# jdeschut/tunempc

Hardware: AMD Instinct MI355X
Metric: stage-Hessian convexifications/sec at (nx+nu)=32, p=64 (higher is better)
Workload: dtype f64

## Files before the change

### tunempc_amd/csrc/tmpc_cr.h

```cpp
#pragma once
#include <climits>
#include <vector>

#include "tmpc_common.h"
#include "tmpc_factor.h"
#include "tmpc_gemm_dma.h"

namespace tmpc {

constexpr int CR_EW = 8;
constexpr int CR_UW = 8;
enum { CE_NODE = 0, CE_NA, CE_NB, CE_EA, CE_EB, CE_FILL, CE_FX, CE_FACC };
enum { CU_NODE = 0, CU_E0, CU_S0, CU_E1, CU_S1 };

struct CrLevel { int eoff, nelim, uoff, nupd; };
struct CrSched {
  int p = 0;
  int prep = 0;
  std::vector<int> orient;
  std::vector<int> elim, upd;
  std::vector<CrLevel> lev;
};

static inline CrSched cr_build(int p) {
// ... 161 lines not shown
  const int* er = cr.elim + (size_t)(eoff + g % nelim) * CR_EW;
  const int which = r / nstrip, strip = r - which * nstrip;
  const int slot = which ? er[CE_EB] : er[CE_EA];
  if (slot < 0) return;
  const int node = er[CE_NODE], dp = dm.dp;
  const size_t bs = (size_t)dp * dp;
  const double* Dk = w.D + ((size_t)b * dm.p + node) * bs;
  const double* Li = w.Linv + ((size_t)b * dm.p + node) * dm.nt * TB * TB;
  const int r0 = strip * rs;
  const int rows = (dp - r0 < rs) ? dp - r0 : rs;
  double* X = cr_edge(w, dm, b, slot) + (size_t)r0 * dp;
  int jt = 0;
  for (int j0 = 0; j0 < dp; j0 += TB, ++jt) {
    const int nb = (dp - j0 < TB) ? dp - j0 : TB;
    if (j0 > 0) wg_gemm_nt<USE_MFMA, 2, 2, 2, NS>(X + j0, dp, X, dp, Dk + (size_t)j0 * dp, dp, rows, nb, j0, GM_SUB, false, lds);
    wg_gemm_nt<USE_MFMA, 2, 2, 2, NS>(X + j0, dp, X + j0, dp, Li + (size_t)jt * TB * TB, TB, rows, nb, nb, GM_SET, false, lds);
  }
}

constexpr int TRR_NT = 5;
__device__ __forceinline__ void vm_wait_le(int n) {
#define TMPC_VMW(K) case K / 2: asm volatile("s_waitcnt vmcnt(" #K ") lgkmcnt(0)" ::: "memory"); break;
  switch (n >> 1) {
    TMPC_VMW(0) TMPC_VMW(2) TMPC_VMW(4) TMPC_VMW(6) TMPC_VMW(8) TMPC_VMW(10) TMPC_VMW(12) TMPC_VMW(14) TMPC_VMW(16) TMPC_VMW(18) TMPC_VMW(20) TMPC_VMW(22)
    default: asm volatile("s_waitcnt vmcnt(24) lgkmcnt(0)" ::: "memory"); break;
  }
#undef TMPC_VMW
}
#ifndef TMPC_TRD_DEPTH
#define TMPC_TRD_DEPTH 2
#endif
constexpr int TRD_DEPTH = TMPC_TRD_DEPTH;
constexpr int trd_lds_doubles() { return 4 * 1024 + TRD_DEPTH * 2048; }
template <bool POTRF>
__device__ __forceinline__ void trd_strip(double* X, const double* Dk, const double* Li, int rows, int nt, int dp, int it, double* lds, float* X32 = nullptr, int ld32 = 0) {
  constexpr int FR = 4, RS = 16 * FR, ASL = RS * 16, DP = TRD_DEPTH;
  int tid = threadIdx.x;
  if (POTRF) asm volatile("" : "+v"(tid));
  const int lane = tid & 63, wv = __builtin_amdgcn_readfirstlane(tid >> 6);
  const int ws = (wv + it) & 3, wc0 = ws * 16;
  const int fk = lane >> 4, fq = (lane >> 2) & 3, fj = lane & 3;
  const int i1 = (rows + 15) >> 4;
  const int nlast = nt - 1, nbl = (dp - 64 * nlast < 64) ? dp - 64 * nlast : 64, ncl = nbl >> 4;
  const int ntd = POTRF ? nt - 1 : nt;
  const bool rw = ws < i1;
  double* At = lds;
  double* Bs = lds + 4 * ASL;
  unsigned voT[2], voL[2];
#pragma unroll
  for (int h = 0; h < 2; ++h) {
    const int row = wv * 16 + 8 * h + (lane >> 3), c = lane & 7;
    voT[h] = (unsigned)(row * TB + 2 * (c ^ dma_sw(row))) * 8u;
    voL[h] = (unsigned)(row * dp + 2 * (c ^ dma_sw(row))) * 8u;
  }
  int oa[2], ob[4][2];
  {
    const int swa = dma_sw(4 * fq + fj);
#pragma unroll
    for (int hh = 0; hh < 2; ++hh) oa[hh] = (4 * fq + fj) * 16 + 2 * ((4 * hh + fk) ^ swa);
#pragma unroll
    for (int e = 0; e < 4; ++e) {
      const int swb = dma_sw(4 * fj + e);
#pragma unroll
      for (int hh = 0; hh < 2; ++hh) ob[e][hh] = (4 * fj + e) * 16 + 2 * ((4 * hh + fk) ^ swb);
    }
  }
  double acc0[4][4], acc1[4][4], acc2[4][4], acc3[4][4];
  int vmtot = 0, vmk0 = 0, vmk1 = 0, vmk2 = 0;
#define TRD_NB(T) ((dp - 64 * (T) < 64) ? dp - 64 * (T) : 64)
// ... 11 lines not shown
    if (on_) vmtot += 2 * i1;                                                                               \
  }
#define TRD_LOAD_R(I, NC, SET)                                                                              \
  {                                                                                                         \
    _Pragma("unroll") for (int c = 0; c < 4; ++c) {                                                          \
      double2_t u0 = (double2_t){0.0, 0.0}, u1 = u0;                                                        \
      if (rw && c < (NC)) {                                                                                 \
        gcptr2 cp = (gcptr2)(X + (size_t)(wc0 + 4 * fq + fk) * dp + 64 * (I) + 16 * c + 4 * fj);            \
        u0 = cp[0]; u1 = cp[1];                                                                             \
      }                                                                                                     \
      SET[c][0] = -u0[0]; SET[c][1] = -u0[1]; SET[c][2] = -u1[0]; SET[c][3] = -u1[1];                       \
    }                                                                                                       \
    if (rw) vmtot += 2 * (NC);                                                                              \
  }
#define TRD_STORE_R(I, NC, SET, SG)                                                                         \
  if (rw) {                                                                                                 \
    _Pragma("unroll") for (int c = 0; c < 4; ++c) {                                                          \
      if (c < (NC)) {                                                                                       \
        typedef double2_t __attribute__((address_space(1)))* gptr2;                                         \
        gptr2 cp = (gptr2)(X + (size_t)(wc0 + 4 * fq + fk) * dp + 64 * (I) + 16 * c + 4 * fj);              \
        if (X32) {       \
          typedef float4_t __attribute__((address_space(1)))* gptr4;                                        \
          *(gptr4)(X32 + (size_t)(wc0 + 4 * fq + fk) * ld32 + 64 * (I) + 16 * c + 4 * fj) =                 \
              (float4_t){(float)(SG SET[c][0]), (float)(SG SET[c][1]), (float)(SG SET[c][2]), (float)(SG SET[c][3])}; \
        } else {                                                                                            \
          cp[0] = (double2_t){SG SET[c][0], SG SET[c][1]}; cp[1] = (double2_t){SG SET[c][2], SG SET[c][3]}; \
        }                                                                                                   \
      }                                                                                                     \
    }                                                                                                       \
    vmtot += (X32 ? 1 : 2) * (NC);                                                                          \
  }
#define TRD_PARK_C(SET)                                                                        \
  {                                                                                                         \
    _Pragma("unroll") for (int i = 0; i < 4; ++i) {                                                          \
      const int row = 16 * i + 4 * fq + fk, sw_ = dma_sw(row);                                              \
      double* q = At + ws * ASL + row * 16;                                                                \
      *(double2_t*)(q + 2 * ((2 * fj) ^ sw_)) = (double2_t){-SET[i][0], -SET[i][1]};                        \
      *(double2_t*)(q + 2 * ((2 * fj + 1) ^ sw_)) = (double2_t){-SET[i][2], -SET[i][3]};                    \
    }                                                                                                       \
  }
#define TRD_PARK_R(NC, SET, SG)                                                                             \
  if (rw) {                                                                                                 \
    const int row = wc0 + 4 * fq + fk, sw_ = dma_sw(row);                                                   \
    _Pragma("unroll") for (int c = 0; c < 4; ++c) {                                                          \
      if (c < (NC)) {                                                                                       \
        double* q = At + c * ASL + row * 16;                                                               \
        *(double2_t*)(q + 2 * ((2 * fj) ^ sw_)) = (double2_t){SG SET[c][0], SG SET[c][1]};                  \
        *(double2_t*)(q + 2 * ((2 * fj + 1) ^ sw_)) = (double2_t){SG SET[c][2], SG SET[c][3]};              \
      }                                                                                                     \
    }                                                                                                       \
  }
#define TRD_ZERO(SET)                                                                                       \
  {                                                                                                         \
    _Pragma("unroll") for (int i = 0; i < 4; ++i)                                                            \
      _Pragma("unroll") for (int c = 0; c < 4; ++c) SET[i][c] = 0.0;                                        \
  }
  int ii = 0, ij = 0, is = 0, nissued = 0, ndone = 0;
#define TRD_ISSUE()           \
  {                                                                                                         \
    if (ii < ntd) {                                                                                         \
      double* dst_ = Bs + (nissued % DP) * 2048 + wv * 256;                                                 \
      const int nsl_ = (ij == ii) ? (TRD_NB(ii) >> 4) : 4;                                                  \
      const bool two_ = 2 * is + 1 < nsl_;                                                                  \
      if (ij == ii) {                                                                                       \
        const int nb_ = TRD_NB(ii);                                                                         \
        const __amdgpu_buffer_rsrc_t rs_ = __builtin_amdgcn_make_buffer_rsrc((void*)(Li + (size_t)ii * TB * TB), 0, (int)(((unsigned)(nb_ - 1) * TB + (unsigned)nb_) * 8u), 0x00020000); \
        __builtin_amdgcn_raw_ptr_buffer_load_lds(rs_, (lds_vptr)(dst_), 16, voT[0], is * 256, 0, 0);        \
        __builtin_amdgcn_raw_ptr_buffer_load_lds(rs_, (lds_vptr)(dst_ + 128), 16, voT[1], is * 256, 0, 0);  \
        if (two_) {                                                                                         \
          __builtin_amdgcn_raw_ptr_buffer_load_lds(rs_, (lds_vptr)(dst_ + 1024), 16, voT[0], is * 256 + 128, 0, 0);       \
          __builtin_amdgcn_raw_ptr_buffer_load_lds(rs_, (lds_vptr)(dst_ + 1024 + 128), 16, voT[1], is * 256 + 128, 0, 0); \
        }                                                                                                   \
      } else {                                                                                              \
        const int nb_ = TRD_NB(ij);                                                                         \
        const __amdgpu_buffer_rsrc_t rs_ = __builtin_amdgcn_make_buffer_rsrc((void*)(Dk + (size_t)(64 * ij) * dp + 64 * ii), 0, (int)(((unsigned)(nb_ - 1) * (unsigned)dp + 64u) * 8u), 0x00020000); \
        __builtin_amdgcn_raw_ptr_buffer_load_lds(rs_, (lds_vptr)(dst_), 16, voL[0], is * 256, 0, 0);        \
        __builtin_amdgcn_raw_ptr_buffer_load_lds(rs_, (lds_vptr)(dst_ + 128), 16, voL[1], is * 256, 0, 0);  \
        __builtin_amdgcn_raw_ptr_buffer_load_lds(rs_, (lds_vptr)(dst_ + 1024), 16, voL[0], is * 256 + 128, 0, 0);         \
        __builtin_amdgcn_raw_ptr_buffer_load_lds(rs_, (lds_vptr)(dst_ + 1024 + 128), 16, voL[1], is * 256 + 128, 0, 0);   \
      }                                                                                                     \
      vmtot += (ij == ii && !two_) ? 2 : 4;                                                                 \
      { const int k_ = nissued % DP; if (k_ == 0) vmk0 = vmtot; else if (k_ == 1) vmk1 = vmtot; else vmk2 = vmtot; }  \
      ++nissued;                                                                                            \
      if (++is == ((nsl_ + 1) >> 1)) { is = 0; if (++ij >= ntd) { ++ii; ij = ii; } }                        \
    }                                                                                                       \
  }
#define TRD_MMA_C(TGT, AS, BS)                                                                              \
  _Pragma("unroll") for (int hh = 0; hh < 2; ++hh) {                                                        \
    double2_t a_[4], b_[4];                                                                                  \
    _Pragma("unroll") for (int i = 0; i < 4; ++i) a_[i] = *(const double2_t*)((AS) + oa[hh] + i * 256);      \
    _Pragma("unroll") for (int cb = 0; cb < 4; ++cb) b_[cb] = *(const double2_t*)((BS) + wc0 * 16 + ob[cb][hh]); \
    _Pragma("unroll") for (int i = 0; i < 4; ++i) {                                                          \
      _Pragma("unroll") for (int cb = 0; cb < 4; ++cb) {                                                    \
        TGT[i][cb] = __builtin_amdgcn_mfma_f64_4x4x4f64(a_[i][0], b_[cb][0], TGT[i][cb], 0, 0, 0);          \
        TGT[i][cb] = __builtin_amdgcn_mfma_f64_4x4x4f64(a_[i][1], b_[cb][1], TGT[i][cb], 0, 0, 0);          \
      }                                                                                                     \
    }                                                                                                       \
  }
#define TRD_MMA_R(TGT, AS, BS, C0, NC)                                                                      \
  _Pragma("unroll") for (int hh = 0; hh < 2; ++hh) {                                                        \
    const double2_t a_ = *(const double2_t*)((AS) + oa[hh] + wc0 * 16);                                     \
    _Pragma("unroll") for (int c = 0; c < 4; ++c) {                                                          \
      if (c >= (C0) && c < (NC)) {                                                                          \
        double2_t b_[4];                                                                                     \
        _Pragma("unroll") for (int cb = 0; cb < 4; ++cb) b_[cb] = *(const double2_t*)((BS) + c * 256 + ob[cb][hh]); \
        _Pragma("unroll") for (int cb = 0; cb < 4; ++cb) {                                                  \
          TGT[c][cb] = __builtin_amdgcn_mfma_f64_4x4x4f64(a_[0], b_[cb][0], TGT[c][cb], 0, 0, 0);           \
          TGT[c][cb] = __builtin_amdgcn_mfma_f64_4x4x4f64(a_[1], b_[cb][1], TGT[c][cb], 0, 0, 0);           \
        }                                                                                                   \
      }                                                                                                     \
    }                                                                                                       \
  }
#define TRD_STEP_C(TGT) { TRD_MMA_C(TGT, A0, Bc) TRD_MMA_C(TGT, A0 + ASL, Bc + 1024) }
#define TRD_STEP_D0(TGT) { TRD_MMA_R(TGT, At, Bc, 0, 4) TRD_MMA_R(TGT, At + ASL, Bc + 1024, 1, 4) }
#define TRD_STEP_D1(TGT) { TRD_MMA_R(TGT, At + 2 * ASL, Bc, 2, 4) TRD_MMA_R(TGT, At + 3 * ASL, Bc + 1024, 3, 4) }
#define TRD_STEP_RL(N) { TRD_MMA_R(acc0, A0, Bc, 0, N) TRD_MMA_R(acc0, A0 + ASL, Bc + 1024, 0, N) }

  __syncthreads();
  TMPC_TC0()
  TRD_ISSUE()
  if (DP > 2) TRD_ISSUE()
  TRD_LOAD_C(0, acc0)
  if (nt > 2) TRD_LOAD_C(1, acc1) else TRD_ZERO(acc1)
  if (nt > 3) TRD_LOAD_C(2, acc2) else TRD_ZERO(acc2)
  if (nt > 4) TRD_LOAD_C(3, acc3) else TRD_ZERO(acc3)
// ... 93 lines not shown
#undef TRD_STEP_C
#undef TRD_MMA_R
#undef TRD_MMA_C
#undef TRD_ISSUE
#undef TRD_ZERO
#undef TRD_PARK_R
#undef TRD_PARK_C
#undef TRD_STORE_R
#undef TRD_LOAD_R
#undef TRD_LOAD_C
#undef TRD_NB
}

__global__ void __launch_bounds__(256, 2) k_cr_trsm_dma(WS w, Dims dm, CrDev cr, int eoff, int nelim, int count) {
  const int dp = dm.dp;
  const int nst = (dp + 63) / 64;
  const int per = 2 * nst;
  const int it = cr_item(count * nelim * per);
  if (it < 0) return;
  extern __shared__ __attribute__((aligned(16))) double lds[];
  const int g = it / per, r = it - g * per;
  const int b = cr.alist[g / nelim];
  const int* er = cr.elim + (size_t)(eoff + g % nelim) * CR_EW;
  const int which = r / nst, strip = r - which * nst;
  const int slot = which ? er[CE_EB] : er[CE_EA];
  if (slot < 0) return;
  const int node = er[CE_NODE];
  const double* Dk = w.D + ((size_t)b * dm.p + node) * (size_t)dp * dp;
  const double* Li = w.Linv + ((size_t)b * dm.p + node) * dm.nt * TB * TB;
  const int r0 = strip * 64;
  const bool lp = cr_lowp(w, b);
  if (lp && (dm.flags & DF_LOWP_TRSM)) return;
  const int ld32 = cr_ld32(dm);
  trd_strip<false>(cr_edge(w, dm, b, slot) + (size_t)r0 * dp, Dk, Li, (dp - r0 < 64) ? dp - r0 : 64, dm.nt, dp, it, lds,
                   lp ? cr_edge32(w, dm, b, slot) + (size_t)r0 * ld32 : nullptr, ld32);
}

constexpr int trf_lds_doubles() { return 2048 + TRD_DEPTH * 2048; }
__device__ __forceinline__ void trf_strip(const double* X, const double* Dk, const double* Li, int rows, int nt, int dp, int it, double* lds, float* X32, int ld32) {
  constexpr int ASL = 64 * 16, DP = TRD_DEPTH;
  const int tid = threadIdx.x;
  const int lane = tid & 63, wv = __builtin_amdgcn_readfirstlane(tid >> 6);
  const int ws = (wv + it) & 3, wc0 = ws * 16;
  const int fk = lane >> 4, fr = lane & 15;
  const int i1 = (rows + 15) >> 4;
  const int nlast = nt - 1, nbl = (dp - 64 * nlast < 64) ? dp - 64 * nlast : 64, ncl = nbl >> 4;
  const int ntd = nt;
  const bool rw = ws < i1;
  float* At = (float*)lds;
  double* Bs = lds + 2048;
  unsigned voT[2], voL[2];
#pragma unroll
  for (int h = 0; h < 2; ++h) {
    const int row = wv * 16 + 8 * h + (lane >> 3), c = lane & 7;
    voT[h] = (unsigned)(row * TB + 2 * (c ^ dma_sw(row))) * 8u;
    voL[h] = (unsigned)(row * dp + 2 * (c ^ dma_sw(row))) * 8u;
  }
  int of[2];
#pragma unroll
  for (int hh = 0; hh < 2; ++hh) of[hh] = fr * 16 + 2 * ((4 * hh + fk) ^ dma_sw(fr));
  const int asw = (fr >> 1) & 3, ofa = fr * 16 + 4 * (fk ^ asw);
  const int opa0 = 4 * ((2 * fk) & 3 ^ asw) + 2 * (fk >> 1), opa1 = 4 * ((2 * fk + 1) & 3 ^ asw) + 2 * (fk >> 1);
  float4_t acc0[4], acc1[4], acc2[4], acc3[4];
  int vmtot = 0, vmk0 = 0, vmk1 = 0, vmk2 = 0;
#define TRF_NB(T) ((dp - 64 * (T) < 64) ? dp - 64 * (T) : 64)
#define TRF_LOAD_C(I, SET)                                                                                  \
  {                                                                                                         \
    const bool on_ = wc0 < TRF_NB(I);                                                                       \
    _Pragma("unroll") for (int i = 0; i < 4; ++i) {                                                          \
      double2_t u0 = (double2_t){0.0, 0.0}, u1 = u0;                                                        \
      if (on_ && i < i1) {                                                                                  \
        gcptr2 cp = (gcptr2)(X + (size_t)(16 * i + fr) * dp + 64 * (I) + wc0 + 4 * fk);                     \
        u0 = cp[0]; u1 = cp[1];                                                                             \
      }                                                                                                     \
      SET[i] = (float4_t){(float)-u0[0], (float)-u0[1], (float)-u1[0], (float)-u1[1]};                      \
    }                                                                                                       \
    if (on_) vmtot += 2 * i1;                                                                               \
  }
#define TRF_LOAD_R(I, NC, SET)                                                                              \
  {                                                                                                         \
    _Pragma("unroll") for (int c = 0; c < 4; ++c) {                                                          \
      double2_t u0 = (double2_t){0.0, 0.0}, u1 = u0;                                                        \
      if (rw && c < (NC)) {                                                                                 \
        gcptr2 cp = (gcptr2)(X + (size_t)(wc0 + fr) * dp + 64 * (I) + 16 * c + 4 * fk);                     \
        u0 = cp[0]; u1 = cp[1];                                                                             \
      }                                                                                                     \
      SET[c] = (float4_t){(float)-u0[0], (float)-u0[1], (float)-u1[0], (float)-u1[1]};                      \
    }                                                                                                       \
    if (rw) vmtot += 2 * (NC);                                                                              \
  }
#define TRF_STORE_R(I, NC, SET)                                                                             \
  if (rw) {                                                                                                 \
    typedef float4_t __attribute__((address_space(1)))* gptr4;                                              \
    _Pragma("unroll") for (int c = 0; c < 4; ++c)                                                            \
      if (c < (NC)) *(gptr4)(X32 + (size_t)(wc0 + fr) * ld32 + 64 * (I) + 16 * c + 4 * fk) = SET[c];        \
    vmtot += (NC);                                                                                          \
  }
#define TRF_PARK_C(SET)                                                                        \
  {                                                                                                         \
    _Pragma("unroll") for (int i = 0; i < 4; ++i) {                                                          \
      float* q = At + ws * ASL + (16 * i + fr) * 16;                                                        \
      *(float2_t*)(q + opa0) = (float2_t){-SET[i][0], -SET[i][1]};                                           \
      *(float2_t*)(q + opa1) = (float2_t){-SET[i][2], -SET[i][3]};                                           \
    }                                                                                                       \
  }
#define TRF_PARK_R(NC, SET, SG)                                                                             \
  if (rw) {                                                                                                 \
    _Pragma("unroll") for (int c = 0; c < 4; ++c) {                                                          \
      if (c < (NC)) {                                                                                       \
        float* q = At + c * ASL + (wc0 + fr) * 16;                                                          \
        *(float2_t*)(q + opa0) = (float2_t){SG SET[c][0], SG SET[c][1]};                                     \
        *(float2_t*)(q + opa1) = (float2_t){SG SET[c][2], SG SET[c][3]};                                     \
      }                                                                                                     \
    }                                                                                                       \
  }
#define TRF_ZERO(SET) { _Pragma("unroll") for (int i = 0; i < 4; ++i) SET[i] = (float4_t){0.f, 0.f, 0.f, 0.f}; }
  int ii = 0, ij = 0, is = 0, nissued = 0, ndone = 0;
#define TRF_ISSUE()                                                       \
  {                                                                                                         \
    if (ii < ntd) {                                                                                         \
      double* dst_ = Bs + (nissued % DP) * 2048 + wv * 256;                                                 \
      const int nsl_ = (ij == ii) ? (TRF_NB(ii) >> 4) : 4;                                                  \
      const bool two_ = 2 * is + 1 < nsl_;                                                                  \
      if (ij == ii) {                                                                                       \
        const int nb_ = TRF_NB(ii);                                                                         \
        const __amdgpu_buffer_rsrc_t rs_ = __builtin_amdgcn_make_buffer_rsrc((void*)(Li + (size_t)ii * TB * TB), 0, (int)(((unsigned)(nb_ - 1) * TB + (unsigned)nb_) * 8u), 0x00020000); \
        __builtin_amdgcn_raw_ptr_buffer_load_lds(rs_, (lds_vptr)(dst_), 16, voT[0], is * 256, 0, 0);        \
        __builtin_amdgcn_raw_ptr_buffer_load_lds(rs_, (lds_vptr)(dst_ + 128), 16, voT[1], is * 256, 0, 0);  \
        if (two_) {                                                                                         \
          __builtin_amdgcn_raw_ptr_buffer_load_lds(rs_, (lds_vptr)(dst_ + 1024), 16, voT[0], is * 256 + 128, 0, 0);       \
          __builtin_amdgcn_raw_ptr_buffer_load_lds(rs_, (lds_vptr)(dst_ + 1024 + 128), 16, voT[1], is * 256 + 128, 0, 0); \
        }                                                                                                   \
      } else {                                                                                              \
        const int nb_ = TRF_NB(ij);                                                                         \
        const __amdgpu_buffer_rsrc_t rs_ = __builtin_amdgcn_make_buffer_rsrc((void*)(Dk + (size_t)(64 * ij) * dp + 64 * ii), 0, (int)(((unsigned)(nb_ - 1) * (unsigned)dp + 64u) * 8u), 0x00020000); \
        __builtin_amdgcn_raw_ptr_buffer_load_lds(rs_, (lds_vptr)(dst_), 16, voL[0], is * 256, 0, 0);        \
        __builtin_amdgcn_raw_ptr_buffer_load_lds(rs_, (lds_vptr)(dst_ + 128), 16, voL[1], is * 256, 0, 0);  \
        __builtin_amdgcn_raw_ptr_buffer_load_lds(rs_, (lds_vptr)(dst_ + 1024), 16, voL[0], is * 256 + 128, 0, 0);         \
        __builtin_amdgcn_raw_ptr_buffer_load_lds(rs_, (lds_vptr)(dst_ + 1024 + 128), 16, voL[1], is * 256 + 128, 0, 0);   \
      }                                                                                                     \
      vmtot += (ij == ii && !two_) ? 2 : 4;                                                                 \
      { const int k_ = nissued % DP; if (k_ == 0) vmk0 = vmtot; else if (k_ == 1) vmk1 = vmtot; else vmk2 = vmtot; }  \
      ++nissued;                                                                                            \
      if (++is == ((nsl_ + 1) >> 1)) { is = 0; if (++ij >= ntd) { ++ii; ij = ii; } }                        \
    }                                                                                                       \
  }
#define TRF_MMA_C(TGT, AS, BS)                                                                              \
  {                                                                                                         \
    float4_t a_[4];                                                                                          \
    _Pragma("unroll") for (int i = 0; i < 4; ++i) a_[i] = *(const float4_t*)((AS) + i * 256 + ofa);         \
    _Pragma("unroll") for (int hh = 0; hh < 2; ++hh) {                                                      \
      const double2_t b_ = *(const double2_t*)((BS) + wc0 * 16 + of[hh]);                                   \
      _Pragma("unroll") for (int e = 0; e < 2; ++e) {                                                        \
        const float bf_ = (float)b_[e];                                                                      \
        _Pragma("unroll") for (int i = 0; i < 4; ++i)                                                        \
          TGT[i] = __builtin_amdgcn_mfma_f32_16x16x4f32(bf_, a_[i][2 * hh + e], TGT[i], 0, 0, 0);           \
      }                                                                                                     \
    }                                                                                                       \
  }
#define TRF_MMA_R(TGT, AS, BS, C0, NC)                                                                      \
  {                                                                                                         \
    const float4_t a_ = *(const float4_t*)((AS) + wc0 * 16 + ofa);                                          \
    _Pragma("unroll") for (int hh = 0; hh < 2; ++hh) {                                                      \
      double2_t b_[4];                                                                                       \
      _Pragma("unroll") for (int c = 0; c < 4; ++c)                                                          \
        if (c >= (C0) && c < (NC)) b_[c] = *(const double2_t*)((BS) + c * 256 + of[hh]);                    \
      _Pragma("unroll") for (int e = 0; e < 2; ++e) {                                                        \
        _Pragma("unroll") for (int c = 0; c < 4; ++c)                                                        \
          if (c >= (C0) && c < (NC)) TGT[c] = __builtin_amdgcn_mfma_f32_16x16x4f32((float)b_[c][e], a_[2 * hh + e], TGT[c], 0, 0, 0); \
      }                                                                                                     \
    }                                                                                                       \
  }
#define TRF_STEP_C(TGT) { TRF_MMA_C(TGT, A0, Bc) TRF_MMA_C(TGT, A0 + ASL, Bc + 1024) }
#define TRF_STEP_D0(TGT) { TRF_MMA_R(TGT, At, Bc, 0, 4) TRF_MMA_R(TGT, At + ASL, Bc + 1024, 1, 4) }
#define TRF_STEP_D1(TGT) { TRF_MMA_R(TGT, At + 2 * ASL, Bc, 2, 4) TRF_MMA_R(TGT, At + 3 * ASL, Bc + 1024, 3, 4) }
#define TRF_STEP_RL(N) { TRF_MMA_R(acc0, A0, Bc, 0, N) TRF_MMA_R(acc0, A0 + ASL, Bc + 1024, 0, N) }

  __syncthreads();
  TRF_ISSUE()
  if (DP > 2) TRF_ISSUE()
  TRF_LOAD_C(0, acc0)
  if (nt > 2) TRF_LOAD_C(1, acc1) else TRF_ZERO(acc1)
  if (nt > 3) TRF_LOAD_C(2, acc2) else TRF_ZERO(acc2)
  if (nt > 4) TRF_LOAD_C(3, acc3) else TRF_ZERO(acc3)
  TRF_PARK_C(acc0)
  TRF_ZERO(acc0)
#define TRF_STEP_BEGIN()                                                                                    \
    { const int k_ = ndone % DP; vm_wait_le(vmtot - (k_ == 0 ? vmk0 : k_ == 1 ? vmk1 : vmk2)); }            \
// ... 60 lines not shown
#undef TRF_STEP_D0
#undef TRF_STEP_C
#undef TRF_MMA_R
#undef TRF_MMA_C
#undef TRF_ISSUE
#undef TRF_ZERO
#undef TRF_PARK_R
#undef TRF_PARK_C
#undef TRF_STORE_R
#undef TRF_LOAD_R
#undef TRF_LOAD_C
#undef TRF_NB
}

__global__ void __launch_bounds__(256, 2) k_cr_trsm_dma_f32(WS w, Dims dm, CrDev cr, int eoff, int nelim, int count) {
  const int dp = dm.dp;
  const int nst = (dp + 63) / 64;
  const int per = 2 * nst;
  const int it = cr_item(count * nelim * per);
  if (it < 0) return;
  extern __shared__ __attribute__((aligned(16))) double lds[];
  const int g = it / per, r = it - g * per;
  const int b = cr.alist[g / nelim];
  if (!cr_lowp(w, b)) return;
  const int* er = cr.elim + (size_t)(eoff + g % nelim) * CR_EW;
  const int which = r / nst, strip = r - which * nst;
  const int slot = which ? er[CE_EB] : er[CE_EA];
  if (slot < 0) return;
  const int node = er[CE_NODE];
  const double* Dk = w.D + ((size_t)b * dm.p + node) * (size_t)dp * dp;
  const double* Li = w.Linv + ((size_t)b * dm.p + node) * dm.nt * TB * TB;
  const int r0 = strip * 64;
  const int ld32 = cr_ld32(dm);
  trf_strip(cr_edge(w, dm, b, slot) + (size_t)r0 * dp, Dk, Li, (dp - r0 < 64) ? dp - r0 : 64, dm.nt, dp, it, lds, cr_edge32(w, dm, b, slot) + (size_t)r0 * ld32, ld32);
}

constexpr int potrf_dma_lds_doubles() { return FACT_LDS_DOUBLES > trd_lds_doubles() ? FACT_LDS_DOUBLES : trd_lds_doubles(); }
__global__ void __launch_bounds__(256, 2) k_cr_potrf_dma(WS w, Dims dm, CrDev cr, int eoff, int nelim, int count) {
  const int it = cr_item(count * nelim);
  if (it < 0) return;
  extern __shared__ __attribute__((aligned(16))) double lds[];
  const int b = cr.alist[it / nelim];
  const int* er = cr.elim + (size_t)(eoff + it % nelim) * CR_EW;
  const int node = er[CE_NODE], dp = dm.dp;
  double* Dk = w.D + ((size_t)b * dm.p + node) * (size_t)dp * dp;
  double* Li = w.Linv + ((size_t)b * dm.p + node) * dm.nt * TB * TB;
  const double* dref = w.Ddiag + ((size_t)b * dm.p + node) * dp;
  double* stat = lds + FACT_LDS_DOUBLES - 8;
  if (threadIdx.x == 0) { stat[0] = 0.0; stat[1] = 1.0; }
  for (int r = 0; r < dm.nt; ++r) {
    const int r0 = 64 * r, nb = (dp - r0 < 64) ? dp - r0 : 64;
    if (r > 0) {
      trd_strip<true>(Dk + (size_t)r0 * dp, Dk, Li, nb, r + 1, dp, it, lds);
      __syncthreads();
    }
    wg_potrf_inv(Dk + (size_t)r0 * dp + r0, dp, Li + (size_t)r * TB * TB, dref + r0, nb, lds, nullptr, stat, (it >> 5) & 3, r > 0);
  }
  if (threadIdx.x == 0) {
    const int nbad = (int)stat[0];
    const double minr = stat[1];
    if (nbad) atomicAdd(w.iprob + (size_t)b * IS + I_NSHIFT, nbad);
    if (w.prob && minr < 1.0) atomic_min_pos(w.prob + (size_t)b * PS + P_MINPIV, minr);
  }
}

template <bool USE_MFMA, int NS>
__global__ void __launch_bounds__(256, 2) k_cr_update(WS w, Dims dm, CrDev cr, int eoff, int nelim, int uoff, int nupd, int count, int mt) {
// ... 110 lines not shown
__global__ void __launch_bounds__(256, 5) k_cr_update_dma_f32(WS w, Dims dm, CrDev cr, int eoff, int nelim, int uoff, int nupd, int count) {
  const int dp = dm.dp;
  const int nm = (dp + 63) / 64;
  const int ntl = nm * (nm + 1) / 2, ntf = nm * nm;
  const int per = nupd * ntl + nelim * ntf;
  const int it = cr_item(count * per);
  if (it < 0) return;
  extern __shared__ __attribute__((aligned(16))) double lds[];
  const int b = cr.alist[it / per];
  if (!cr_lowp(w, b)) return;
  const int r = it % per;
  const size_t bs = (size_t)dp * dp;
  const int slot_items = ntf + ntl, ld32 = cr_ld32(dm);
  int j = r / slot_items, rr = r - j * slot_items;
  bool is_upd;
  {
    const int nmin = nelim < nupd ? nelim : nupd;
    const int full = nmin * slot_items;
    if (r < full) { is_upd = rr >= ntf; if (is_upd) rr -= ntf; }
    else if (nelim > nupd) { const int q = r - full; j = nmin + q / ntf; rr = q % ntf; is_upd = false; }
    else { const int q = r - full; j = nmin + q / ntl; rr = q % ntl; is_upd = true; }
  }
  if (is_upd) {
    const int* ur = cr.upd + (size_t)(uoff + (j + 1) % nupd) * CR_UW;
    int t = rr, tm = 0;
    while (t > tm) { t -= tm + 1; ++tm; }
    const int tn = t;
    const int m0 = tm * 64, n0 = tn * 64;
    const int M = (dp - m0 < 64) ? dp - m0 : 64, N = (dp - n0 < 64) ? dp - n0 : 64;
    double* C = w.D + ((size_t)b * dm.p + ur[CU_NODE]) * bs + (size_t)m0 * dp + n0;
    const float* P0 = cr_edge32(w, dm, b, ur[CU_E0]);
    const float* P1 = ur[CU_E1] >= 0 ? cr_edge32(w, dm, b, ur[CU_E1]) : nullptr;
    wg_tile_dma_f32<UPD_DMA_DEPTH>(C, dp, P0 + (size_t)m0 * ld32, P0 + (size_t)n0 * ld32, P1 ? P1 + (size_t)m0 * ld32 : nullptr, P1 ? P1 + (size_t)n0 * ld32 : nullptr,
                                   ld32, M, N, ld32, GM_SUB, tm == tn ? 0 : GM_NOTRI, it, lds, TMPC_ABL(dm));
  } else {
    const int* er = cr.elim + (size_t)(eoff + j) * CR_EW;
    if (er[CE_FILL] < 0) return;
    const int tm = rr / nm, tn = rr - tm * nm;
    const int m0 = tm * 64, n0 = tn * 64;
    const int M = (dp - m0 < 64) ? dp - m0 : 64, N = (dp - n0 < 64) ? dp - n0 : 64;
    const float* Px = cr_edge32(w, dm, b, er[CE_FX] ? er[CE_EB] : er[CE_EA]);
    const float* Py = cr_edge32(w, dm, b, er[CE_FX] ? er[CE_EA] : er[CE_EB]);
    double* C = cr_edge(w, dm, b, er[CE_FILL]) + (size_t)m0 * dp + n0;
    wg_tile_dma_f32<UPD_DMA_DEPTH>(C, dp, Px + (size_t)m0 * ld32, Py + (size_t)n0 * ld32, nullptr, nullptr, ld32, M, N, ld32, er[CE_FACC] ? GM_SUB : GM_NEG, GM_NOTRI, it, lds, TMPC_ABL(dm));
  }
}

constexpr int NCV = 3;
constexpr int cr_solve_lds_doubles(int dp) { return 2 * NCV * (dp + 4) + NCP * (TB + 4) + 64 * GLDV + 16; }

__global__ void __launch_bounds__(256) k_cr_fwd_diag(WS w, Dims dm, CrDev cr, int eoff, int nelim, int count, int pass) {
  const int it = cr_item(count * nelim);
  if (it < 0) return;
  extern __shared__ __attribute__((aligned(16))) double lds[];
  const int b = cr.alist[it / nelim];
  const int nc = cr_nc(w, b, pass);
  if (nc == 0) return;
  const int* er = cr.elim + (size_t)(eoff + it % nelim) * CR_EW;
  const int node = er[CE_NODE], dp = dm.dp, xld = dp + 4, tld = TB + 4;
  double* zc = lds; double* tmp = lds + 2 * NCV * xld; double* As = tmp + NCP * tld;
  for (int e = threadIdx.x; e < NCV * xld; e += 256) zc[e] = 0.0;
  for (int e = threadIdx.x; e < NCP * tld; e += 256) tmp[e] = 0.0;
  __syncthreads();
  double* R = cr_rhs(w, dm, b, node, nc);
  vec_g2s(zc, xld, R, dp, nc);
  __syncthreads();
  blk_fwd(zc, xld, tmp, tld, w.D + ((size_t)b * dm.p + node) * dp * dp, w.Linv + ((size_t)b * dm.p + node) * dm.nt * TB * TB, dp, As, nc);
  vec_s2g(R, zc, xld, dp, nc);
}

__global__ void __launch_bounds__(256) k_cr_fwd_off(WS w, Dims dm, CrDev cr, int uoff, int nupd, int count, int pass, int lowp_only) {
  const int it = cr_item(count * nupd);
  if (it < 0) return;
  extern __shared__ __attribute__((aligned(16))) double lds[];
  const int b = cr.alist[it / nupd];
  if (lowp_only && !cr_lowp(w, b)) return;
  const int nc = cr_nc(w, b, pass);
// ... 50 lines not shown
```

### tunempc_amd/csrc/tmpc_gemm_dma.h

```cpp
#pragma once
#include "tmpc_common.h"
#include "tmpc_factor.h"

namespace tmpc {

typedef __attribute__((address_space(3))) void* lds_vptr;
constexpr int DMA_SLAB = 2048;
template <int DEPTH>
constexpr int dma_lds_doubles() { return DEPTH * DMA_SLAB + 512; }

__device__ __forceinline__ int dma_sw(int r) { return (r & 7) ^ (((r >> 3) & 1) << 1); }

template <int DEPTH, bool ZFUSE = false>
__device__ __forceinline__ void wg_tile_dma(double* C, int ldc, const double* A0, const double* B0, const double* A1, const double* B1, int ld,
                                            int M, int N, int K, int mode, int tri, int rot, double* lds, int ldb = 0,
                                            const double* z0 = nullptr, const double* z1 = nullptr, double* yz = nullptr, int znc = 0) {
  if (ldb == 0) ldb = ld;
  const int tid = threadIdx.x, lane = tid & 63, wv = tid >> 6;
  const int wc0 = ((wv + rot) & 3) * 16;
  const int fk = lane >> 4, fq = (lane >> 2) & 3, fj = lane & 3;
  const bool wave_on = wc0 < N;
  int i0 = 0;
  if (tri != GM_NOTRI) { i0 = (tri + wc0) >> 4; if (i0 < 0) i0 = 0; }
  const int i1 = (M + 15) >> 4;
// ... 110 lines not shown
    double yv[4];
#pragma unroll
    for (int i = 0; i < 4; ++i) yv[i] = (i < i1) ? yz[(size_t)(16 * i + 4 * fq + fk) * znc + fj] : 0.0;
#pragma unroll
    for (int i = 0; i < 4; ++i)
      if (i < i1) yz[(size_t)(16 * i + 4 * fq + fk) * znc + fj] = yv[i] - accz[i];
  }
  if (wave_on) {
    typedef double2_t __attribute__((address_space(1)))* gptr2;
    double2_t cu[4][2];
#pragma unroll
    for (int i = 0; i < 4; ++i) {
      cu[i][0] = (double2_t){0.0, 0.0}; cu[i][1] = cu[i][0];
      if (mode == GM_SUB && i >= i0 && i < i1) {
        gcptr2 cq = (gcptr2)(C + (size_t)(16 * i + 4 * fq + fk) * ldc + wc0 + 4 * fj);
        cu[i][0] = cq[0]; cu[i][1] = cq[1];
      }
    }
#pragma unroll
    for (int i = 0; i < 4; ++i) {
      if (i >= i0 && i < i1) {
        gptr2 cp = (gptr2)(C + (size_t)(16 * i + 4 * fq + fk) * ldc + wc0 + 4 * fj);
        double2_t u0 = cu[i][0], u1 = cu[i][1];
        if (mode == GM_SET) { u0[0] = acc[i][0]; u0[1] = acc[i][1]; u1[0] = acc[i][2]; u1[1] = acc[i][3]; }
        else { u0[0] -= acc[i][0]; u0[1] -= acc[i][1]; u1[0] -= acc[i][2]; u1[1] -= acc[i][3]; }
        cp[0] = u0; cp[1] = u1;
      }
    }
  }
}

template <int DEPTH>
__device__ __forceinline__ void wg_tile_dma_f32(double* C, int ldc, const float* A0, const float* B0, const float* A1, const float* B1, int ld32,
                                                int M, int N, int K32, int mode, int tri, int rot, double* lds, int ablate = 0) {
  const int tid = threadIdx.x, lane = tid & 63, wv = __builtin_amdgcn_readfirstlane(tid >> 6);
  const int wc0 = ((wv + rot) & 3) * 16;
  const int fk = lane >> 4, fr = lane & 15;
  const bool wave_on = wc0 < N;
  int i0 = 0;
  if (tri != GM_NOTRI) { i0 = (tri + wc0) >> 4; if (i0 < 0) i0 = 0; }
  const int i1 = (M + 15) >> 4;
  const unsigned abytes = ((unsigned)(M - 1) * (unsigned)ld32 + (unsigned)K32) * 4u, bbytes = ((unsigned)(N - 1) * (unsigned)ld32 + (unsigned)K32) * 4u;
  const __amdgpu_buffer_rsrc_t ra0 = __builtin_amdgcn_make_buffer_rsrc((void*)A0, 0, (int)abytes, 0x00020000);
  const __amdgpu_buffer_rsrc_t rb0 = __builtin_amdgcn_make_buffer_rsrc((void*)B0, 0, (int)bbytes, 0x00020000);
  const __amdgpu_buffer_rsrc_t ra1 = __builtin_amdgcn_make_buffer_rsrc((void*)(A1 ? A1 : A0), 0, (int)abytes, 0x00020000);
  const __amdgpu_buffer_rsrc_t rb1 = __builtin_amdgcn_make_buffer_rsrc((void*)(B1 ? B1 : B0), 0, (int)bbytes, 0x00020000);
  unsigned vo[2];
#pragma unroll
  for (int h = 0; h < 2; ++h) {
    const int row = wv * 16 + 8 * h + (lane >> 3), c = lane & 7;
    vo[h] = (unsigned)(row * ld32 * 4 + 16 * (c ^ dma_sw(row)));
  }
  int oa[2], ob[2];
#pragma unroll
  for (int hh = 0; hh < 2; ++hh) {
    oa[hh] = fr * 16 + 2 * ((4 * hh + fk) ^ dma_sw(fr));
    ob[hh] = (wc0 + fr) * 16 + 2 * ((4 * hh + fk) ^ dma_sw(wc0 + fr));
  }
  float4_t acc[4];
#pragma unroll
  for (int i = 0; i < 4; ++i) acc[i] = (float4_t){0.f, 0.f, 0.f, 0.f};
  const int nks = K32 >> 5, nst = A1 ? 2 * nks : nks;
  const int frange = wave_on ? (i0 * 8 + i1) : -1;
#define TMPC_DMAF_ISSUE(S, Q)                                                                             \
  {                                                                                                       \
    double* As_ = lds + (Q) * DMA_SLAB;                                                                   \
    const bool second_ = (S) >= nks;                                                                      \
    const int so_ = ((S) - (second_ ? nks : 0)) * 128;                                                    \
    _Pragma("unroll") for (int h = 0; h < 2; ++h) {                                                       \
      if (second_) {                                                                                      \
        __builtin_amdgcn_raw_ptr_buffer_load_lds(ra1, (lds_vptr)(As_ + (wv * 16 + 8 * h) * 16), 16, vo[h], so_, 0, 0);        \
        __builtin_amdgcn_raw_ptr_buffer_load_lds(rb1, (lds_vptr)(As_ + 1024 + (wv * 16 + 8 * h) * 16), 16, vo[h], so_, 0, 0); \
      } else {                                                                                            \
        __builtin_amdgcn_raw_ptr_buffer_load_lds(ra0, (lds_vptr)(As_ + (wv * 16 + 8 * h) * 16), 16, vo[h], so_, 0, 0);        \
        __builtin_amdgcn_raw_ptr_buffer_load_lds(rb0, (lds_vptr)(As_ + 1024 + (wv * 16 + 8 * h) * 16), 16, vo[h], so_, 0, 0); \
      }                                                                                                   \
    }                                                                                                     \
  }
#define TMPC_DMAF_MMA(I0, I1)                                                                             \
  _Pragma("unroll") for (int hh = 0; hh < 2; ++hh) {                                                      \
    float4_t a[4];                                                                                        \
    _Pragma("unroll") for (int i = (I0); i < (I1); ++i) a[i] = *(const float4_t*)(As_ + oa[hh] + i * 256); \
    const float4_t bv = *(const float4_t*)(Bs_ + ob[hh]);                                                 \
    _Pragma("unroll") for (int e = 0; e < 4; ++e) {                                                       \
      _Pragma("unroll") for (int i = (I0); i < (I1); ++i) {                                               \
        if (ablate != 2) acc[i] = __builtin_amdgcn_mfma_f32_16x16x4f32(a[i][e], bv[e], acc[i], 0, 0, 0);  \
      }                                                                                                   \
    }                                                                                                     \
  }
#define TMPC_DMAF_MMA_DISPATCH()                                                                          \
  switch (frange) {                                                                                       \
    case 0 * 8 + 4: TMPC_DMAF_MMA(0, 4) break;  case 1 * 8 + 4: TMPC_DMAF_MMA(1, 4) break;                \
    case 2 * 8 + 4: TMPC_DMAF_MMA(2, 4) break;  case 3 * 8 + 4: TMPC_DMAF_MMA(3, 4) break;                \
    case 0 * 8 + 3: TMPC_DMAF_MMA(0, 3) break;  case 1 * 8 + 3: TMPC_DMAF_MMA(1, 3) break;                \
    case 2 * 8 + 3: TMPC_DMAF_MMA(2, 3) break;                                                            \
    case 0 * 8 + 2: TMPC_DMAF_MMA(0, 2) break;  case 1 * 8 + 2: TMPC_DMAF_MMA(1, 2) break;                \
    case 0 * 8 + 1: TMPC_DMAF_MMA(0, 1) break;                                                            \
    default: break;                                                                                       \
  }
#define TMPC_DMAF_STEP(S, Q)                                                                              \
  {                                                                                                       \
    if ((S) + DEPTH - 2 < nst - 1) { asm volatile("s_waitcnt vmcnt(%0) lgkmcnt(0)" ::"n"(4 * (DEPTH - 2)) : "memory"); } \
    else { asm volatile("s_waitcnt vmcnt(0) lgkmcnt(0)" ::: "memory"); }                                  \
    if (ablate != 4) __builtin_amdgcn_s_barrier();                                                        \
    if ((S) + DEPTH - 1 < nst && ablate != 3) TMPC_DMAF_ISSUE((S) + DEPTH - 1, ((Q) + DEPTH - 1) % DEPTH) \
    const double* As_ = lds + (Q) * DMA_SLAB;                                                             \
    const double* Bs_ = As_ + 1024;                                                                       \
    TMPC_DMAF_MMA_DISPATCH()                                                                              \
  }
  __syncthreads();
#pragma unroll
  for (int s = 0; s < DEPTH - 1; ++s)
    if (s < nst) TMPC_DMAF_ISSUE(s, s)
  for (int s = 0; s < nst; s += DEPTH) {
#pragma unroll
    for (int q = 0; q < DEPTH; ++q)
      if (s + q < nst) TMPC_DMAF_STEP(s + q, q)
  }
#undef TMPC_DMAF_STEP
#undef TMPC_DMAF_MMA_DISPATCH
#undef TMPC_DMAF_MMA
#undef TMPC_DMAF_ISSUE
  if (ablate == 1) { if (acc[0][0] == 123.456f) C[0] = 1.0; return; }
  if (wave_on) {
    double cu[4][4];
#pragma unroll
    for (int i = 0; i < 4; ++i)
#pragma unroll
      for (int r = 0; r < 4; ++r) {
        cu[i][r] = 0.0;
        if (mode == GM_SUB && i >= i0 && i < i1) cu[i][r] = C[(size_t)(16 * i + 4 * fk + r) * ldc + wc0 + fr];
      }
#pragma unroll
    for (int i = 0; i < 4; ++i)
      if (i >= i0 && i < i1) {
#pragma unroll
        for (int r = 0; r < 4; ++r) C[(size_t)(16 * i + 4 * fk + r) * ldc + wc0 + fr] = (mode == GM_SET) ? (double)acc[i][r] : cu[i][r] - (double)acc[i][r];
      }
  }
}
// ... 4 lines not shown
```

### tunempc_amd/csrc/tmpc_schur.h

```cpp
#pragma once
#include "tmpc_common.h"
#include "tmpc_small.h"

namespace tmpc {

#ifndef TMPC_POLISH_ENTER
#define TMPC_POLISH_ENTER 1e-4
#endif
constexpr double POLISH_ENTER_GPU = TMPC_POLISH_ENTER;
constexpr int MUT_BACKOFF_MAX = 10;

constexpr int SCH_NT = 320;
template <int PART> constexpr int sch_rec() { return PART == 0 ? 10 : 6; }
__device__ __forceinline__ double hkm_t(double xac, double xad, double xbc, double xbd, double sac, double sad, double sbc, double sbd) {
  return (xac * sbd + xad * sbc) + (xbc * sad + xbd * sac);
}
template <int PART, bool GF, int NTS>
__device__ __forceinline__ void schur_body(const WS& w, const Dims& dm, int sid, int tid, double* sm) {
  constexpr int REC = sch_rec<PART>();
  const int b = sid / dm.p, k = sid - b * dm.p;
  const int* ip = w.iprob + (size_t)b * IS;
  if (ip[I_PHASE] == PH_DONE) return;
  const int nx = dm.nx, nxx = nx * nx, d = dm.d, dp = dm.dp;
  const int reg = ip[I_REG];
  const double regf = (reg <= 0) ? 1.0 : 1.0 + 1e-13 * ((reg == 1) ? 10.0 : (reg == 2) ? 100.0 : 1000.0);
  double* mats = GF ? w.sscr + (size_t)sid * 10 * nxx : sm;
  unsigned* pair = (unsigned*)(GF ? sm : sm + (size_t)nxx * REC);
  const bool corner = (w.cr_orient[k] != 0);
  const int km = (k == 0) ? dm.p - 1 : k - 1;
  const double* kfk = w.KF + (size_t)sid * 12 * nxx;
  const double* kfm = w.KF + (size_t)(b * dm.p + km) * 12 * nxx;
  for (int e = tid; e < 12 * nxx; e += NTS) {
    const int m = e / nxx, r = e - m * nxx;
    const int lmi = m / KF_PER_LMI, slot = m - lmi * KF_PER_LMI;
    const bool fmat = (slot == KF_FX || slot == KF_FS);
    if (fmat != (PART == 1)) continue;
    const double v = (slot == KF_KX || slot == KF_KS) ? kfm[e] : kfk[e];
    int i = r / nx, j = r - i * nx;
    if (fmat && !corner) { const int t_ = i; i = j; j = t_; }
    const int q = fmat ? 2 * lmi + (slot - KF_FX) : 4 * lmi + slot;
    mats[(size_t)(i * nx + j) * REC + q] = v;
  }
  if (tid < nx) {
    int e = tid * nx - (tid * (tid - 1)) / 2;
    for (int c = tid; c < nx; ++c) pair[e++] = (unsigned)tid | ((unsigned)c << 16);
  }
  if (NTS == 64) asm volatile("s_waitcnt vmcnt(0) lgkmcnt(0)" ::: "memory");
  else __syncthreads();
  double* Dg = w.D + (size_t)sid * dp * dp;
  double* Cg = w.O + (size_t)sid * dp * dp;
  double* dd = w.Ddiag + (size_t)sid * dp;
  for (int col = tid; col < dp; col += NTS) {
    const bool cin = col < d;
    const unsigned pc_ = cin ? pair[col] : 0u;
    const int c = (int)(pc_ & 0xffffu), d_ = (int)(pc_ >> 16);
    const double wc = (c == d_) ? 0.5 : 1.0;
    const double2_t* rc = (const double2_t*)(mats + (size_t)c * REC);
    const double2_t* rd = (const double2_t*)(mats + (size_t)d_ * REC);
    constexpr int NQ = PART == 0 ? 4 : 2;
    double2_t ac[NQ], ad[NQ];
    int a_prev = -1;
    const int row0 = (PART == 0) ? (col / 64) * 64 : 0;
    for (int row = row0; row < dp; ++row) {
      const size_t e = (size_t)row * dp + col;
      if (row >= d || !cin) {
        if (PART == 0) { if (col <= row) Dg[e] = (row == col) ? 1.0 : 0.0; if (row == col) dd[row] = 1.0; }
        else Cg[e] = 0.0;
        continue;
      }
      const unsigned pr_ = (unsigned)__builtin_amdgcn_readfirstlane((int)pair[row]);
      const int a = (int)(pr_ & 0xffffu), bb = (int)(pr_ >> 16);
      const int ro = nx * (REC / 2);
      if (a != a_prev) {
        a_prev = a;
#pragma unroll
        for (int q = 0; q < NQ; ++q) { ac[q] = rc[a * ro + q]; ad[q] = rd[a * ro + q]; }
      }
      const double wgt = ((a == bb) ? 0.5 : 1.0) * wc;
      if (PART == 1) {
        const double2_t bc0 = rc[bb * ro], bd0 = rd[bb * ro], bc1 = rc[bb * ro + 1], bd1 = rd[bb * ro + 1];
        double cv = 0.0;
        cv -= wgt * hkm_t(ac[0][0], ad[0][0], bc0[0], bd0[0], ac[0][1], ad[0][1], bc0[1], bd0[1]);
        cv -= wgt * hkm_t(ac[1][0], ad[1][0], bc1[0], bd1[0], ac[1][1], ad[1][1], bc1[1], bd1[1]);
        Cg[e] = cv;
      } else if (col <= row) {
        double dv = 0.0;
#pragma unroll
        for (int r = 0; r < 2; ++r) {
          const double2_t bc0 = rc[bb * ro + 2 * r], bd0 = rd[bb * ro + 2 * r];
          const double2_t bc1 = rc[bb * ro + 2 * r + 1], bd1 = rd[bb * ro + 2 * r + 1];
          dv += wgt * hkm_t(ac[2 * r][0], ad[2 * r][0], bc0[0], bd0[0], ac[2 * r][1], ad[2 * r][1], bc0[1], bd0[1]);
          dv += wgt * hkm_t(ac[2 * r + 1][0], ad[2 * r + 1][0], bc1[0], bd1[0], ac[2 * r + 1][1], ad[2 * r + 1][1], bc1[1], bd1[1]);
        }
        if (row == col) { dv *= regf; dd[row] = dv; }
        Dg[e] = dv;
      }
    }
  }
}

template <int PART, bool GF = false>
__global__ void __launch_bounds__(SCH_NT) k_schur(WS w, Dims dm) {
  extern __shared__ __attribute__((aligned(16))) double sm[];
  schur_body<PART, GF, SCH_NT>(w, dm, stage_id(w, dm), threadIdx.x, sm);
}

__device__ __forceinline__ void gather_body(const WS& w, const Dims& dm, int sid, int lane, int pass) {
  const int b = sid / dm.p, k = sid - b * dm.p;
  const int* ip = w.iprob + (size_t)b * IS;
  const int phase = ip[I_PHASE];
  if (phase == PH_DONE) return;
  if (pass == 1 && phase != PH_MAIN) return;
  const bool three = (pass == 1) || (phase != PH_MAIN && !ip[I_CHORD]);
  const int nx = dm.nx, nxx = nx * nx, dp = dm.dp;
  const int km = (k == 0) ? dm.p - 1 : k - 1;
  const double* av = w.adjV + (size_t)(b * dm.p + km) * NADJ * nxx;
  const double* ae = w.adjE + (size_t)sid * NADJ * nxx;
  int e = 0;
  for (int a = 0; a < nx; ++a) {
    for (int c = a + lane; c < nx; c += 64) {
      const int idx = e + (c - a);
      const double wgt = (a == c) ? 1.0 : 2.0;
      const int o = a * nx + c;
      const double g = wgt * (av[ADJ_G * nxx + o] - ae[ADJ_G * nxx + o]);
      if (three) {
        const double ut = -wgt * (av[ADJ_PSI * nxx + o] - ae[ADJ_PSI * nxx + o]);
        const double ua = wgt * (av[ADJ_PHI * nxx + o] - ae[ADJ_PHI * nxx + o]);
        double* w3 = w.W3 + ((size_t)sid * dp + idx) * 3;
        w3[0] = g; w3[1] = ut; w3[2] = ua;
        double* u = w.U + ((size_t)sid * dp + idx) * 2;
// ... 284 lines not shown
```

Measured before the change: 12250.

## Trim padded work in TRSM strips, f32 update K loop, and Schur tile walk

Templates the double and float triangular-solve strip kernels on the row-fragment count and uses three fragments when a strip has 48 or fewer rows, which skips MFMA and LDS work on padded rows. The f32 DMA update GEMM now receives the true K, rounds it up internally, and skips the second half-step when K is an odd multiple of 16. The Schur PART 0 kernel now assigns lower-triangular 64x64 tiles to waves instead of whole columns to threads, which balances the triangular fill across waves. More template instantiations raise code size, and the half-K path depends on correct padding semantics.

```diff
diff --git a/tunempc_amd/csrc/tmpc_cr.h b/tunempc_amd/csrc/tmpc_cr.h
--- a/tunempc_amd/csrc/tmpc_cr.h
+++ b/tunempc_amd/csrc/tmpc_cr.h
@@ -217,9 +217,9 @@
 #endif
 constexpr int TRD_DEPTH = TMPC_TRD_DEPTH;
 constexpr int trd_lds_doubles() { return 4 * 1024 + TRD_DEPTH * 2048; }
-template <bool POTRF>
+template <bool POTRF, int FR = 4>
 __device__ __forceinline__ void trd_strip(double* X, const double* Dk, const double* Li, int rows, int nt, int dp, int it, double* lds, float* X32 = nullptr, int ld32 = 0) {
-  constexpr int FR = 4, RS = 16 * FR, ASL = RS * 16, DP = TRD_DEPTH;
+  constexpr int ASL = 64 * 16, DP = TRD_DEPTH;
   int tid = threadIdx.x;
   if (POTRF) asm volatile("" : "+v"(tid));
   const int lane = tid & 63, wv = __builtin_amdgcn_readfirstlane(tid >> 6);
@@ -297,7 +297,7 @@
   }
 #define TRD_PARK_C(SET)                                                                        \
   {                                                                                                         \
-    _Pragma("unroll") for (int i = 0; i < 4; ++i) {                                                          \
+    _Pragma("unroll") for (int i = 0; i < FR; ++i) {                                                         \
       const int row = 16 * i + 4 * fq + fk, sw_ = dma_sw(row);                                              \
       double* q = At + ws * ASL + row * 16;                                                                \
       *(double2_t*)(q + 2 * ((2 * fj) ^ sw_)) = (double2_t){-SET[i][0], -SET[i][1]};                        \
@@ -353,9 +353,9 @@
 #define TRD_MMA_C(TGT, AS, BS)                                                                              \
   _Pragma("unroll") for (int hh = 0; hh < 2; ++hh) {                                                        \
     double2_t a_[4], b_[4];                                                                                  \
-    _Pragma("unroll") for (int i = 0; i < 4; ++i) a_[i] = *(const double2_t*)((AS) + oa[hh] + i * 256);      \
+    _Pragma("unroll") for (int i = 0; i < FR; ++i) a_[i] = *(const double2_t*)((AS) + oa[hh] + i * 256);     \
     _Pragma("unroll") for (int cb = 0; cb < 4; ++cb) b_[cb] = *(const double2_t*)((BS) + wc0 * 16 + ob[cb][hh]); \
-    _Pragma("unroll") for (int i = 0; i < 4; ++i) {                                                          \
+    _Pragma("unroll") for (int i = 0; i < FR; ++i) {                                                         \
       _Pragma("unroll") for (int cb = 0; cb < 4; ++cb) {                                                    \
         TGT[i][cb] = __builtin_amdgcn_mfma_f64_4x4x4f64(a_[i][0], b_[cb][0], TGT[i][cb], 0, 0, 0);          \
         TGT[i][cb] = __builtin_amdgcn_mfma_f64_4x4x4f64(a_[i][1], b_[cb][1], TGT[i][cb], 0, 0, 0);          \
@@ -515,11 +515,15 @@
   const bool lp = cr_lowp(w, b);
   if (lp && (dm.flags & DF_LOWP_TRSM)) return;
   const int ld32 = cr_ld32(dm);
-  trd_strip<false>(cr_edge(w, dm, b, slot) + (size_t)r0 * dp, Dk, Li, (dp - r0 < 64) ? dp - r0 : 64, dm.nt, dp, it, lds,
-                   lp ? cr_edge32(w, dm, b, slot) + (size_t)r0 * ld32 : nullptr, ld32);
+  const int rows = (dp - r0 < 64) ? dp - r0 : 64;
+  double* X = cr_edge(w, dm, b, slot) + (size_t)r0 * dp;
+  float* X32 = lp ? cr_edge32(w, dm, b, slot) + (size_t)r0 * ld32 : nullptr;
+  if (rows <= 48) trd_strip<false, 3>(X, Dk, Li, rows, dm.nt, dp, it, lds, X32, ld32);
+  else trd_strip<false, 4>(X, Dk, Li, rows, dm.nt, dp, it, lds, X32, ld32);
 }
 
 constexpr int trf_lds_doubles() { return 2048 + TRD_DEPTH * 2048; }
+template <int FR = 4>
 __device__ __forceinline__ void trf_strip(const double* X, const double* Dk, const double* Li, int rows, int nt, int dp, int it, double* lds, float* X32, int ld32) {
   constexpr int ASL = 64 * 16, DP = TRD_DEPTH;
   const int tid = threadIdx.x;
@@ -581,7 +585,7 @@
   }
 #define TRF_PARK_C(SET)                                                                        \
   {                                                                                                         \
-    _Pragma("unroll") for (int i = 0; i < 4; ++i) {                                                          \
+    _Pragma("unroll") for (int i = 0; i < FR; ++i) {                                                         \
       float* q = At + ws * ASL + (16 * i + fr) * 16;                                                        \
       *(float2_t*)(q + opa0) = (float2_t){-SET[i][0], -SET[i][1]};                                           \
       *(float2_t*)(q + opa1) = (float2_t){-SET[i][2], -SET[i][3]};                                           \
@@ -631,12 +635,12 @@
 #define TRF_MMA_C(TGT, AS, BS)                                                                              \
   {                                                                                                         \
     float4_t a_[4];                                                                                          \
-    _Pragma("unroll") for (int i = 0; i < 4; ++i) a_[i] = *(const float4_t*)((AS) + i * 256 + ofa);         \
+    _Pragma("unroll") for (int i = 0; i < FR; ++i) a_[i] = *(const float4_t*)((AS) + i * 256 + ofa);        \
     _Pragma("unroll") for (int hh = 0; hh < 2; ++hh) {                                                      \
       const double2_t b_ = *(const double2_t*)((BS) + wc0 * 16 + of[hh]);                                   \
       _Pragma("unroll") for (int e = 0; e < 2; ++e) {                                                        \
         const float bf_ = (float)b_[e];                                                                      \
-        _Pragma("unroll") for (int i = 0; i < 4; ++i)                                                        \
+        _Pragma("unroll") for (int i = 0; i < FR; ++i)                                                       \
           TGT[i] = __builtin_amdgcn_mfma_f32_16x16x4f32(bf_, a_[i][2 * hh + e], TGT[i], 0, 0, 0);           \
       }                                                                                                     \
     }                                                                                                       \
@@ -763,7 +767,11 @@
   const double* Li = w.Linv + ((size_t)b * dm.p + node) * dm.nt * TB * TB;
   const int r0 = strip * 64;
   const int ld32 = cr_ld32(dm);
-  trf_strip(cr_edge(w, dm, b, slot) + (size_t)r0 * dp, Dk, Li, (dp - r0 < 64) ? dp - r0 : 64, dm.nt, dp, it, lds, cr_edge32(w, dm, b, slot) + (size_t)r0 * ld32, ld32);
+  const int rows = (dp - r0 < 64) ? dp - r0 : 64;
+  const double* X = cr_edge(w, dm, b, slot) + (size_t)r0 * dp;
+  float* X32 = cr_edge32(w, dm, b, slot) + (size_t)r0 * ld32;
+  if (rows <= 48) trf_strip<3>(X, Dk, Li, rows, dm.nt, dp, it, lds, X32, ld32);
+  else trf_strip<4>(X, Dk, Li, rows, dm.nt, dp, it, lds, X32, ld32);
 }
 
 constexpr int potrf_dma_lds_doubles() { return FACT_LDS_DOUBLES > trd_lds_doubles() ? FACT_LDS_DOUBLES : trd_lds_doubles(); }
@@ -940,7 +948,7 @@
     const float* P0 = cr_edge32(w, dm, b, ur[CU_E0]);
     const float* P1 = ur[CU_E1] >= 0 ? cr_edge32(w, dm, b, ur[CU_E1]) : nullptr;
     wg_tile_dma_f32<UPD_DMA_DEPTH>(C, dp, P0 + (size_t)m0 * ld32, P0 + (size_t)n0 * ld32, P1 ? P1 + (size_t)m0 * ld32 : nullptr, P1 ? P1 + (size_t)n0 * ld32 : nullptr,
-                                   ld32, M, N, ld32, GM_SUB, tm == tn ? 0 : GM_NOTRI, it, lds, TMPC_ABL(dm));
+                                   ld32, M, N, dp, GM_SUB, tm == tn ? 0 : GM_NOTRI, it, lds, TMPC_ABL(dm));
   } else {
     const int* er = cr.elim + (size_t)(eoff + j) * CR_EW;
     if (er[CE_FILL] < 0) return;
@@ -950,7 +958,7 @@
     const float* Px = cr_edge32(w, dm, b, er[CE_FX] ? er[CE_EB] : er[CE_EA]);
     const float* Py = cr_edge32(w, dm, b, er[CE_FX] ? er[CE_EA] : er[CE_EB]);
     double* C = cr_edge(w, dm, b, er[CE_FILL]) + (size_t)m0 * dp + n0;
-    wg_tile_dma_f32<UPD_DMA_DEPTH>(C, dp, Px + (size_t)m0 * ld32, Py + (size_t)n0 * ld32, nullptr, nullptr, ld32, M, N, ld32, er[CE_FACC] ? GM_SUB : GM_NEG, GM_NOTRI, it, lds, TMPC_ABL(dm));
+    wg_tile_dma_f32<UPD_DMA_DEPTH>(C, dp, Px + (size_t)m0 * ld32, Py + (size_t)n0 * ld32, nullptr, nullptr, ld32, M, N, dp, er[CE_FACC] ? GM_SUB : GM_NEG, GM_NOTRI, it, lds, TMPC_ABL(dm));
   }
 }
 
diff --git a/tunempc_amd/csrc/tmpc_gemm_dma.h b/tunempc_amd/csrc/tmpc_gemm_dma.h
--- a/tunempc_amd/csrc/tmpc_gemm_dma.h
+++ b/tunempc_amd/csrc/tmpc_gemm_dma.h
@@ -166,7 +166,7 @@
 
 template <int DEPTH>
 __device__ __forceinline__ void wg_tile_dma_f32(double* C, int ldc, const float* A0, const float* B0, const float* A1, const float* B1, int ld32,
-                                                int M, int N, int K32, int mode, int tri, int rot, double* lds, int ablate = 0) {
+                                                int M, int N, int K, int mode, int tri, int rot, double* lds, int ablate = 0) {
   const int tid = threadIdx.x, lane = tid & 63, wv = __builtin_amdgcn_readfirstlane(tid >> 6);
   const int wc0 = ((wv + rot) & 3) * 16;
   const int fk = lane >> 4, fr = lane & 15;
@@ -174,6 +174,7 @@
   int i0 = 0;
   if (tri != GM_NOTRI) { i0 = (tri + wc0) >> 4; if (i0 < 0) i0 = 0; }
   const int i1 = (M + 15) >> 4;
+  const int K32 = (K + 31) & ~31;
   const unsigned abytes = ((unsigned)(M - 1) * (unsigned)ld32 + (unsigned)K32) * 4u, bbytes = ((unsigned)(N - 1) * (unsigned)ld32 + (unsigned)K32) * 4u;
   const __amdgpu_buffer_rsrc_t ra0 = __builtin_amdgcn_make_buffer_rsrc((void*)A0, 0, (int)abytes, 0x00020000);
   const __amdgpu_buffer_rsrc_t rb0 = __builtin_amdgcn_make_buffer_rsrc((void*)B0, 0, (int)bbytes, 0x00020000);
@@ -195,6 +196,7 @@
 #pragma unroll
   for (int i = 0; i < 4; ++i) acc[i] = (float4_t){0.f, 0.f, 0.f, 0.f};
   const int nks = K32 >> 5, nst = A1 ? 2 * nks : nks;
+  const bool khalf = (K & 16) != 0;
   const int frange = wave_on ? (i0 * 8 + i1) : -1;
 #define TMPC_DMAF_ISSUE(S, Q)                                                                             \
   {                                                                                                       \
@@ -213,12 +215,14 @@
   }
 #define TMPC_DMAF_MMA(I0, I1)                                                                             \
   _Pragma("unroll") for (int hh = 0; hh < 2; ++hh) {                                                      \
-    float4_t a[4];                                                                                        \
-    _Pragma("unroll") for (int i = (I0); i < (I1); ++i) a[i] = *(const float4_t*)(As_ + oa[hh] + i * 256); \
-    const float4_t bv = *(const float4_t*)(Bs_ + ob[hh]);                                                 \
-    _Pragma("unroll") for (int e = 0; e < 4; ++e) {                                                       \
-      _Pragma("unroll") for (int i = (I0); i < (I1); ++i) {                                               \
-        if (ablate != 2) acc[i] = __builtin_amdgcn_mfma_f32_16x16x4f32(a[i][e], bv[e], acc[i], 0, 0, 0);  \
+    if (hh == 0 || !half_) {                             \
+      float4_t a[4];                                                                                      \
+      _Pragma("unroll") for (int i = (I0); i < (I1); ++i) a[i] = *(const float4_t*)(As_ + oa[hh] + i * 256); \
+      const float4_t bv = *(const float4_t*)(Bs_ + ob[hh]);                                               \
+      _Pragma("unroll") for (int e = 0; e < 4; ++e) {                                                     \
+        _Pragma("unroll") for (int i = (I0); i < (I1); ++i) {                                             \
+          if (ablate != 2) acc[i] = __builtin_amdgcn_mfma_f32_16x16x4f32(a[i][e], bv[e], acc[i], 0, 0, 0); \
+        }                                                                                                 \
       }                                                                                                   \
     }                                                                                                     \
   }
@@ -240,6 +244,7 @@
     if ((S) + DEPTH - 1 < nst && ablate != 3) TMPC_DMAF_ISSUE((S) + DEPTH - 1, ((Q) + DEPTH - 1) % DEPTH) \
     const double* As_ = lds + (Q) * DMA_SLAB;                                                             \
     const double* Bs_ = As_ + 1024;                                                                       \
+    const bool half_ = khalf && ((S) == nks - 1 || (S) == nst - 1);                                       \
     TMPC_DMAF_MMA_DISPATCH()                                                                              \
   }
   __syncthreads();
diff --git a/tunempc_amd/csrc/tmpc_schur.h b/tunempc_amd/csrc/tmpc_schur.h
--- a/tunempc_amd/csrc/tmpc_schur.h
+++ b/tunempc_amd/csrc/tmpc_schur.h
@@ -50,7 +50,7 @@
   double* Dg = w.D + (size_t)sid * dp * dp;
   double* Cg = w.O + (size_t)sid * dp * dp;
   double* dd = w.Ddiag + (size_t)sid * dp;
-  for (int col = tid; col < dp; col += NTS) {
+  auto walk = [&](const int col, const int rbeg, const int rend) {
     const bool cin = col < d;
     const unsigned pc_ = cin ? pair[col] : 0u;
     const int c = (int)(pc_ & 0xffffu), d_ = (int)(pc_ >> 16);
@@ -60,8 +60,7 @@
     constexpr int NQ = PART == 0 ? 4 : 2;
     double2_t ac[NQ], ad[NQ];
     int a_prev = -1;
-    const int row0 = (PART == 0) ? (col / 64) * 64 : 0;
-    for (int row = row0; row < dp; ++row) {
+    for (int row = rbeg; row < rend; ++row) {
       const size_t e = (size_t)row * dp + col;
       if (row >= d || !cin) {
         if (PART == 0) { if (col <= row) Dg[e] = (row == col) ? 1.0 : 0.0; if (row == col) dd[row] = 1.0; }
@@ -96,6 +95,19 @@
         Dg[e] = dv;
       }
     }
+  };
+  if (PART == 0) {
+    constexpr int NW = NTS / 64;
+    const int wv = __builtin_amdgcn_readfirstlane(tid >> 6), lane = tid & 63;
+    const int nct = (dp + 63) >> 6, nun = nct * (nct + 1) / 2;
+    for (int u = wv; u < nun; u += NW) {
+      int r = 0, c = u;
+      while (c > r) { c -= r + 1; ++r; }
+      const int col = 64 * c + lane, rend = (64 * r + 64 < dp) ? 64 * r + 64 : dp;
+      if (col < dp) walk(col, 64 * r, rend);
+    }
+  } else {
+    for (int col = tid; col < dp; col += NTS) walk(col, 0, dp);
   }
 }
 
```

After: 12350 (median of 6 runs). No clear change (+0.8%).
